# RFD-FHEM/PySignalduino

Measured on AMD Instinct MI355X. Metric: RF messages/sec demodulated (MU+MS+MC, full protocol bank), higher is better.
Workload: dtype u8+f64; 1 GPU; mixed MU/MS/MC stream, 1/3 each per rank: MU 256-pulse messages x 129-id MU bank, MS sync+bits x 66-id MS bank (clock x U(0.6,1.4)), MC frames x 12 clockrange ids ('fixed' chain); kind=mixed, corpus=bench, msgs_per_gpu=1000000, batches=3, input_bytes_resident=571611860, parallelism=dp1, grouped=True, streams=one kernel (k_step: MU, then MS, then MC tiles)

## Files before the change

### pysignalduino_amd/csrc/sdx_kernels.hip

```cpp
#include "sdx_device.h"
#include "sdx_lane.h"
#include "sdx_mc.h"

#include <atomic>
#include <cstdio>
#include <cstring>
#include <mutex>
#include <string>
#include <type_traits>

#ifdef SDX_WGTIME
__device__ unsigned long long g_wgt[2 * 65536];
#endif
#ifdef SDX_PROF
__device__ unsigned long long g_prof[32];
__device__ unsigned long long g_gprof[2][128];
#define PROF_T(v) unsigned long long v = __builtin_amdgcn_s_memtime()
#define PROF_ADD(slot, v)                                                                   \
  do {                                                                                      \
    if (__lane_id() == 0) L.prof[wave][slot] += (unsigned)(__builtin_amdgcn_s_memtime() - (v)); \
  } while (0)
#define PROF_CNT(slot, x)                                                                   \
  do {                                                                                      \
    if (__lane_id() == 0) L.prof[wave][slot] += (unsigned)(x);                              \
  } while (0)
#define PROF_ADDD(slot, v)                                                                  \
  do {                                                                                      \
    if (__lane_id() == __ffsll((unsigned long long)__builtin_amdgcn_read_exec()) - 1)       \
      L.prof[wave][slot] += (unsigned)(__builtin_amdgcn_s_memtime() - (v));                 \
  } while (0)
#define PROF_CNTL(slot) atomicAdd(&L.prof[wave][slot], 1u)
#else
#define PROF_T(v)
#define PROF_ADD(slot, v)
#define PROF_ADDD(slot, v)
#define PROF_CNT(slot, x)
#define PROF_CNTL(slot)
#endif

#ifndef SDX_NO_RAISE_CHECK
#define SDX_NO_RAISE_CHECK 1
#endif

namespace sdx {

constexpr int POOL_REC = 640;
constexpr int POOL_HEAP = 16384;
constexpr int POOL_REC_MS = 256;
constexpr int POOL_HEAP_MS = 8192;

struct StageRec {
  uint32_t off;
  uint16_t len, proto;
  uint32_t bitlen;
  uint8_t msg, wave;
  uint16_t rank;
};
constexpr uint32_t STAGE_NIB = 0x80000000u;
SDX_DEV uint32_t stage_bitlen(int bitlen, int hex_digits, int pre_len) {
  return (hex_digits >= 0 && hex_digits < 32768 && pre_len <= 255 && (uint32_t)bitlen < 65536u)
             ? (STAGE_NIB | ((uint32_t)hex_digits << 16) | (uint32_t)bitlen)
             : (uint32_t)bitlen;
}

struct MuItem {
  uint32_t st_lo, st_hi;
  uint16_t u0, u1, u2;
  uint16_t idx, p;
  uint8_t mi, fmask;
};
constexpr int QCAP = 128;
#ifndef SDX_LANE_WAVES
#define SDX_LANE_WAVES 8
#endif
constexpr int LANE_WAVES = SDX_LANE_WAVES;

struct MsItem {
  uint32_t k0_lo, k0_hi;
  uint16_t k1, k2, k3;
  uint16_t start;
  uint16_t p;
  uint8_t mi, fmask;
};
constexpr int MS_SURV_CAP = 1024;
constexpr int MS_DESC_LDS = 96;
struct MsDesc {
  int32_t lir_min, lir_max, pad, pre_off, post_off;
  uint16_t pre_len, post_len;
  uint8_t width, klen[4], recon, postdemo, res;
};
static_assert(sizeof(MsDesc) == 32, "MsDesc layout");

struct MuMatch {
  uint16_t q, k;
  uint16_t u0, u1, u2;
  uint16_t p;
  uint8_t mi;
  uint8_t flags;
  uint8_t j;
};
constexpr int MATCH_CAP = 768;

constexpr uint32_t SPILL_M = 2048, SPILL_R = 2048, SPILL_H = 49152;
constexpr uint32_t SPILL_OFF_R = SPILL_M * 16, SPILL_OFF_H = SPILL_OFF_R + SPILL_R * 16;
constexpr uint32_t SPILL_BYTES = SPILL_OFF_H + SPILL_H;
constexpr uint32_t SPILL_NONE = 0xFFFFFFFFu, SPILL_PENDING = 0xFFFFFFFEu, SPILL_FULL = 0xFFFFFFFDu;
constexpr uint32_t HEAP_SPILLED = 0x80000000u;
constexpr uint8_t REC_HOLE = 0xFF;
static_assert(sizeof(MuMatch) == 16, "MuMatch spill layout");

template <int NW, int TM, int LM>
struct TileLds {
  static constexpr int WS = NW;
  static constexpr int MSTRIDE = 10 * NW + 1;
  static constexpr int NBITS = 64 * NW + 64;
  struct Wave {
    uint64_t umask[3][NW];
    uint64_t uany[NW];
    uint64_t smask[NW];
    uint64_t stream[NW + 18];
    uint8_t bits[NBITS];
    uint8_t bits2[NBITS];
  };
  uint64_t bm[TM * MSTRIDE];
  uint64_t pairs[TM][2];
  int32_t nlen[TM];
  uint32_t raise_key[TM];
  uint32_t digit_ok[TM];
  uint32_t cnt[TM];
  uint32_t rec_base, heap_base, tile_bad, tot_rec;
  uint32_t mbase[TM];
  struct WaveScratch4 {
    Wave w[4];
  };
  struct NoScratch {};
  typename std::conditional<LM != 0, NoScratch, WaveScratch4>::type wa;
  static constexpr int PREC = LM == 1 ? 512 : (NW <= 4 ? POOL_REC_MS * (TM > 64 ? 2 : 1) : POOL_REC);
  static constexpr int PHEAP =
      LM == 1 ? 10240 : (NW <= 4 ? POOL_HEAP_MS * (TM > 64 ? 2 : 1) : POOL_HEAP);
  static constexpr int SCAP = TM > 64 ? MS_SURV_CAP + MS_SURV_CAP / 4 : MS_SURV_CAP;
  static constexpr int NHALF = (LM == 2 && TM > 64) ? 2 : 1;
  static_assert(TM <= 64 * NHALF, "one lane per message of a half");
  StageRec rec[PREC];
  alignas(16) uint8_t heap[PHEAP];
  unsigned long long pool_ctr;
  uint32_t spill_base, sp_rec, sp_heap;
  int ovf, next_p[NHALF];
  int mm_states, nmatch;
  MuMatch mlist[LM == 1 ? MATCH_CAP : 1];
  alignas(16) sdx_mu_desc desc[LM == 1 ? SDX_MUDESC_LDS : 1];
  union alignas(16) {
    MuItem q[LM == 1 ? LANE_WAVES : 1][LM == 1 ? QCAP : 1];
    uint8_t mmtab[LM == 1 ? SDX_MMTAB_LDS : 16];
  } u;
  MsItem slist[LM == 2 ? SCAP : 1];
  int nsurv;
  MsDesc msdesc[LM == 2 ? MS_DESC_LDS : 1];
#ifdef SDX_PROF
  unsigned int prof[LM != 0 ? LANE_WAVES : 4][28];
#endif
};

SDX_DEV void wave_sync() {
  __builtin_amdgcn_fence(__ATOMIC_SEQ_CST, "wavefront");
  __builtin_amdgcn_wave_barrier();
}

SDX_DEV int lanes_below(uint64_t mask) {
  const int l = lane_id();
  return popc64(l ? (mask & ((1ull << l) - 1)) : 0ull);
}

template <class T>
SDX_DEV int pool_alloc(T& L, int total, int* rec_slot) {
  int h = -1, r = -1;
  if (lane_id() == 0) {
    const unsigned long long o = atomicAdd(&L.pool_ctr, ((unsigned long long)total << 32) | 1ull);
    r = (int)(uint32_t)o;
    h = (int)(o >> 32);
    if (r >= T::PREC || h + total > T::PHEAP) {
      L.ovf = 1;
      h = -1;
    }
  }
  h = bcast_i(h, 0);
  *rec_slot = bcast_i(r, 0);
  return h;
}

template <class T>
SDX_DEV void pool_commit(T& L, int slot, int wave, int msg_local, int proto, int off, int total, int bitlen) {
  if (lane_id() == 0) {
    StageRec r;
    r.off = (uint32_t)off;
    r.len = (uint16_t)total;
    r.proto = (uint16_t)proto;
    r.bitlen = (uint32_t)bitlen;
    r.msg = (uint8_t)msg_local;
    r.wave = (uint8_t)wave;
    r.rank = (uint16_t)atomicAdd(&L.cnt[msg_local], 1u);
    L.rec[slot] = r;
  }
  wave_sync();
}

template <class T>
SDX_DEV uint32_t spill_region(T& L, const sdx_out& out) {
  uint32_t b = __hip_atomic_load(&L.spill_base, __ATOMIC_RELAXED, __HIP_MEMORY_SCOPE_WORKGROUP);
  if (b >= SPILL_PENDING) {
    const int leader = ffs64(ballot(true));
    if (lane_id() == leader) {
      uint32_t cur = atomicCAS(&L.spill_base, SPILL_NONE, SPILL_PENDING);
      if (cur == SPILL_NONE) {
        const uint32_t idx = atomicAdd(&out.cursor_dev[3], 1u);
        const uint64_t o = (uint64_t)idx * SPILL_BYTES;
        cur = (out.work_dev && o + SPILL_BYTES <= out.work_cap) ? (uint32_t)o : SPILL_FULL;
        __hip_atomic_store(&L.spill_base, cur, __ATOMIC_RELAXED, __HIP_MEMORY_SCOPE_WORKGROUP);
      }
      while (cur == SPILL_PENDING) cur = __hip_atomic_load(&L.spill_base, __ATOMIC_RELAXED, __HIP_MEMORY_SCOPE_WORKGROUP);
      b = cur;
    }
    b = (uint32_t)__shfl((int)b, leader);
  }
  if (b == SPILL_FULL || !out.work_dev || (uint64_t)b + SPILL_BYTES > out.work_cap) return SPILL_NONE;
  return b;
}

struct PoolSlot {
  StageRec* rec;
  uint8_t* heap;
  uint32_t off;
};
template <class T>
SDX_DEV bool pool_take(T& L, const sdx_out& out, int span, PoolSlot* ps) {
  const unsigned long long o = atomicAdd(&L.pool_ctr, ((unsigned long long)span << 32) | 1ull);
  const int slot = (int)(uint32_t)o, off = (int)(o >> 32);
  if (slot < T::PREC && off + span <= T::PHEAP) {
    ps->rec = &L.rec[slot];
    ps->heap = L.heap + off;
    ps->off = (uint32_t)off;
    return true;
  }
  if (slot < T::PREC) L.rec[slot].msg = REC_HOLE;
  const uint32_t base = spill_region(L, out);
  const uint32_t rs = atomicAdd(&L.sp_rec, 1u), hs = atomicAdd(&L.sp_heap, (uint32_t)span);
  if (base == SPILL_NONE || rs >= SPILL_R || hs + (uint32_t)span > SPILL_H) {
    L.ovf = 1;
    return false;
  }
  uint8_t* reg = out.work_dev + base;
  ps->rec = reinterpret_cast<StageRec*>(reg + SPILL_OFF_R) + rs;
  ps->heap = reg + SPILL_OFF_H + hs;
  ps->off = HEAP_SPILLED | hs;
  return true;
}

SDX_DEV void copy_str(uint8_t* dst, const uint8_t* src, int n) {
  for (int i = lane_id(); i < n; i += WAVE) dst[i] = src[i];
}

SDX_DEV int any_float(const uint8_t* bits, int nb) {
  bool f = false;
  for (int i = lane_id(); i < nb; i += WAVE) f |= bits[i] == 2;
  return ballot(f) != 0;
}

SDX_DEV int hex_digits(const uint8_t* bits, int nb, uint8_t* dst, int strip_zero) {
  const int nd = (nb + 3) >> 2;
  int skip = 0;
  if (strip_zero) {
    skip = nd;
    for (int d0 = 0; d0 < nd; d0 += WAVE) {
      const int d = d0 + lane_id();
      int v = 0;
      if (d < nd) {
        const int e = nb - 4 * (nd - 1 - d), a = (e - 4 > 0) ? e - 4 : 0;
        for (int i = a; i < e; ++i) v = (v << 1) | bits[i];
      }
      const uint64_t nz = ballot(d < nd && v != 0);
      if (nz) {
        skip = d0 + ffs64(nz);
        break;
      }
    }
  }
  for (int d = skip + lane_id(); d < nd; d += WAVE) {
    const int e = nb - 4 * (nd - 1 - d), a = (e - 4 > 0) ? e - 4 : 0;
    int v = 0;
    for (int i = a; i < e; ++i) v = (v << 1) | bits[i];
    dst[d - skip] = (uint8_t)(v < 10 ? '0' + v : 'A' + v - 10);
  }
  return nd - skip;
}

template <class T>
SDX_DEV void raise_msg(T& L, int msg_local, int proto, int kind) {
  if (lane_id() == 0) atomicMin(&L.raise_key[msg_local], ((uint32_t)proto << 8) | (uint32_t)kind);
  wave_sync();
}

template <int NW, int TM, int LM>
SDX_DEV void finish_mu(TileLds<NW, TM, LM>& L, int wave, const BankView& bv, const sdx_mu_proto* rec, int p, int s,
                       int nb) {
  auto& W = L.wa.w[wave];
  uint8_t* buf = W.bits;
  PROF_T(t_pd);
  if (cld(&rec->postdemo) != SDX_PD_NONE && !any_float(buf, nb)) {
    int rc = 0, no = 0;
    if (lane_id() == 0) rc = run_postdemo(cld(&rec->postdemo), buf, nb, W.bits2, &no);
    rc = bcast_i(rc, 0);
    no = bcast_i(no, 0);
    wave_sync();
    if (rc == 0) return;
    if (rc == 1) {
      buf = W.bits2;
      nb = no;
    }
  }
  PROF_ADD(7, t_pd);
  PROF_T(t_fmt);
  const int pad = cld(&rec->pad_bits);
  int nbp = nb;
  nbp = (nbp + pad - 1) / pad * pad;
  for (int i = nb + lane_id(); i < nbp; i += WAVE) buf[i] = 0;
  wave_sync();
  const bool isf = any_float(buf, nbp);
  int dlen;
  if (cld(&rec->dispatch_bin)) dlen = nbp;
  else if (isf) {
    if (cld(&rec->remove_zero)) {
      raise_msg(L, s, p, SDX_RAISE_ATTRIBUTE);
      return;
    }
    dlen = 4;
  } else {
    dlen = -2;
  }
  const int nd = (nbp + 3) >> 2;
  int skip = 0;
  if (dlen == -2) {
    if (cld(&rec->remove_zero)) {
      skip = nd;
      for (int d0 = 0; d0 < nd; d0 += WAVE) {
        const int d = d0 + lane_id();
        int v = 0;
        if (d < nd) {
          const int e = nbp - 4 * (nd - 1 - d), a = (e - 4 > 0) ? e - 4 : 0;
          for (int i = a; i < e; ++i) v = (v << 1) | buf[i];
        }
        const uint64_t nz = ballot(d < nd && v != 0);
        if (nz) {
          skip = d0 + ffs64(nz);
          break;
        }
      }
    }
    dlen = nd - skip;
  }
  auto dchar = [&](int d) -> uint8_t {
    if (cld(&rec->dispatch_bin)) return buf[d] == 2 ? 'F' : (uint8_t)('0' + buf[d]);
    if (isf) return (uint8_t)"None"[d];
    const int dd = d + skip, e = nbp - 4 * (nd - 1 - dd), a = (e - 4 > 0) ? e - 4 : 0;
    int v = 0;
    for (int i = a; i < e; ++i) v = (v << 1) | buf[i];
    return (uint8_t)(v < 10 ? '0' + v : 'A' + v - 10);
  };
  if (cld(&rec->mm_dfa) >= 0) {
    int ok = 0;
    if (lane_id() == 0) {
      const sdx_dfa D = bv.dfa[cld(&rec->mm_dfa)];
      const uint8_t* t256 = bv.t256 + D.t256_off;
      const uint8_t* fl = bv.dflags + D.flags_off;
      int st = cld(&rec->mm_pre_state);
      const int tot = dlen + cld(&rec->post_len);
      int i = 0;
      for (; i < tot; ++i) {
        const uint8_t f = fl[st];
        if (f & 5) break;
        const uint8_t c = i < dlen ? dchar(i) : bv.str[cld(&rec->post_off) + i - dlen];
        st = t256[st * 256 + c];
      }
      const uint8_t f = fl[st];
      ok = (f & 1) ? 1 : ((f & 4) ? 0 : ((i == tot && (f & 2)) ? 1 : 0));
    }
    PROF_ADD(9, t_fmt);
    if (!bcast_i(ok, 0)) return;
  }
  PROF_T(t_wr);
  const int total = cld(&rec->pre_len) + dlen + cld(&rec->post_len);
  int slot;
  const int off = pool_alloc(L, total, &slot);
  if (off < 0) return;
  uint8_t* dst = L.heap + off;
  copy_str(dst, bv.str + cld(&rec->pre_off), cld(&rec->pre_len));
  for (int d = lane_id(); d < dlen; d += WAVE) dst[cld(&rec->pre_len) + d] = dchar(d);
  copy_str(dst + cld(&rec->pre_len) + dlen, bv.str + cld(&rec->post_off), cld(&rec->post_len));
  pool_commit(L, slot, wave, s, p, off, total, (int)stage_bitlen(nbp, isf ? -1 : dlen, cld(&rec->pre_len)));
  PROF_ADD(8, t_wr);
  PROF_CNT(20, 1);
}

template <int NW, int TM, int LM>
SDX_DEV void decode_mu(TileLds<NW, TM, LM>& L, int wave, const BankView& bv, const sdx_mu_proto* rec, int p, int s,
                       int idx, uint64_t st_tgt, uint64_t ut0, uint64_t ut1, uint64_t ut2, int fmask) {
  using T = TileLds<NW, TM, LM>;
  auto& W = L.wa.w[wave];
  const int lane = lane_id();
  const uint64_t* bm = &L.bm[s * T::MSTRIDE];
  const int n = L.nlen[s], nw = (n + 63) >> 6;
  const int Lw = cld(&rec->width);
  const int lenS = cld(&rec->has_start) ? (int)cld(&rec->start.len) : 0;
  const uint64_t ut[3] = {ut0, ut1, ut2};
  const uint8_t SYM[3] = {1, 0, 2};
  PROF_T(t_setup);
  PROF_CNT(21, 1);
  uint64_t uni[3] = {0, 0, 0};
  uint8_t usym[3] = {0, 0, 0};
  int nu = 0;
  for (int k = 0; k < 3; ++k) {
    if (!((fmask >> k) & 1)) continue;
    int j = 0;
    for (; j < nu; ++j)
      if (uni[j] == ut[k]) break;
    if (j == nu) uni[nu++] = ut[k];
    usym[j] = SYM[k];
  }
  uint64_t ek[3] = {0, 0, 0};
  uint8_t esym[3] = {0, 0, 0};
  int ne = 0;
  if (cld(&rec->recon) && Lw > 1) {
    const uint64_t msk = (Lw - 1 >= 16) ? ~0ull : ((1ull << (4 * (Lw - 1))) - 1);
    for (int k = 0; k < 3; ++k) {
      if (!((fmask >> k) & 1)) continue;
      const uint64_t key = ut[k] & msk;
      int j = 0;
      for (; j < ne; ++j)
        if (ek[j] == key) break;
      if (j == ne) {
        ek[ne] = key;
        esym[ne] = SYM[k];
        ++ne;
      }
    }
  }
  if (lane < nw) {
    uint64_t any = 0;
    for (int j = 0; j < nu; ++j) {
      uint64_t m = ~0ull;
      for (int i = 0; i < Lw; ++i) {
        const int id = (int)((uni[j] >> (4 * i)) & 15), wo = lane + (i >> 6);
        m &= (wo < nw) ? bm_window(bm + id * T::WS, wo, i & 63, nw) : 0ull;
      }
      W.umask[j][lane] = m;
      any |= m;
    }
    W.uany[lane] = any;
    uint64_t sm = ~0ull;
    for (int i = 0; i < lenS; ++i) {
      const int id = (int)((st_tgt >> (4 * i)) & 15), wo = lane + (i >> 6);
      sm &= (wo < nw) ? bm_window(bm + id * T::WS, wo, i & 63, nw) : 0ull;
    }
    W.smask[lane] = sm;
  }
  wave_sync();
  const int nunits = (n + Lw - 1) / Lw;
  const int sw = (nunits + 63) >> 6;
  for (int r = 0; r < Lw; ++r) {
    for (int c = 0; c < sw; ++c) {
      const int x = r + (c * 64 + lane) * Lw;
      const bool b = x < n && ((W.uany[x >> 6] >> (x & 63)) & 1ull);
// ... 785 lines not shown
  __syncthreads();
  const uint32_t nh_l16 = ((uint32_t)nh_l + 15u) & ~15u;
  constexpr int MPL = (TM + 63) / 64;
  if (tid < 64) {
    const int lane = tid;
    uint32_t cm[MPL], c = 0;
#pragma unroll
    for (int k = 0; k < MPL; ++k) {
      const int m = lane * MPL + k;
      const bool live = !ovf && m < TM && m < nvalid && L.raise_key[m] == 0xFFFFFFFFu;
      cm[k] = live ? cntm[m] : 0u;
      c += cm[k];
    }
    uint32_t x = c;
#pragma unroll
    for (int o = 1; o < 64; o <<= 1) {
      const uint32_t y = __shfl_up(x, o);
      if (lane >= o) x += y;
    }
    uint32_t mb = x - c;
#pragma unroll
    for (int k = 0; k < MPL; ++k) {
      const int m = lane * MPL + k;
      if (m < TM && m < nvalid) L.mbase[m] = mb;
      mb += cm[k];
    }
    const uint32_t nrec = __shfl(x, 63);
    const uint32_t nheap = ovf ? 0u : nh_l16 + (((uint32_t)nh_s + 15u) & ~15u);
    uint32_t got = 0;
    if (!ovf && lane < 2) got = atomicAdd(&out.cursor_dev[lane], lane == 0 ? nrec : nheap);
    const uint32_t rb = __shfl(got, 0), hb = __shfl(got, 1);
    if (lane == 0) {
      int bad = ovf ? 1 : 0;
      if (!bad) {
        if (rb + nrec > out.rec_cap || hb + nheap > out.heap_cap) {
          bad = 2;
          atomicOr(&out.cursor_dev[2], 1u);
        }
      } else {
        atomicOr(&out.cursor_dev[2], 2u);
      }
      L.tile_bad = bad;
      L.rec_base = rb;
      L.heap_base = hb;
      L.tot_rec = nrec;
    }
  }
  __syncthreads();
  const int bad = L.tile_bad;
  if (!bad) {
    for (int r = tid; r < nr; r += blockDim.x) {
      const int m = rec_at(r).msg;
      if (m == REC_HOLE || L.raise_key[m] != 0xFFFFFFFFu) continue;
      const uint32_t b = atomicAdd(&fill[m], 1u);
      bidx[L.mbase[m] + b] = (uint16_t)r;
    }
    __syncthreads();
    const int nt = (int)L.tot_rec;
    for (int j = tid; j < nt; j += blockDim.x) {
      const StageRec sr = rec_at(bidx[j]);
      const uint32_t key = ((uint32_t)sr.proto << 16) | sr.rank;
      const uint32_t b0 = L.mbase[sr.msg], b1 = b0 + cntm[sr.msg];
      uint32_t rk = 0;
      for (uint32_t i = b0; i < b1; ++i) {
        const StageRec o = rec_at(bidx[i]);
        rk += (((uint32_t)o.proto << 16) | o.rank) < key ? 1u : 0u;
      }
      sdx_result o;
      o.payload_off = L.heap_base + ((sr.off & HEAP_SPILLED) ? nh_l16 + (sr.off & ~HEAP_SPILLED) : sr.off);
      o.payload_len = sr.len;
      o.proto = sr.proto;
      const bool staged_nib = (sr.bitlen & STAGE_NIB) != 0;
      o.bit_length = staged_nib ? (sr.bitlen & 0xFFFFu) : sr.bitlen;
      o.msg = (uint32_t)msg_of[sr.msg];
      out.rec_dev[L.rec_base + b0 + rk] = o;
      if (wx) {
        uint32_t xr;
        if (staged_nib) {
          const int pl = kind == SDX_KIND_MU ? bv.mu[sr.proto].pre_len : bv.ms[sr.proto].pre_len;
          xr = SDX_XREC_NIB | ((uint32_t)pl << 16) | ((sr.bitlen >> 16) & 0x7FFFu);
        } else if (sr.off & HEAP_SPILLED) {
          xr = wire_class(bv, kind, sr.proto, sreg + SPILL_OFF_H + (sr.off & ~HEAP_SPILLED), sr.len);
        } else {
          xr = wire_class(bv, kind, sr.proto, L.heap + sr.off, sr.len);
        }
        if (out.xrec_dev) out.xrec_dev[L.rec_base + b0 + rk] = xr;
        atomicAdd(reinterpret_cast<unsigned long long*>(&wsum[sr.msg]),
                  (unsigned long long)(((uint64_t)sr.len << 32) | wire_bytes_x(xr, sr.len)));
      }
    }
    uint8_t* hd = out.heap_dev + L.heap_base;
    if ((((uintptr_t)hd) & 15u) == 0) {
      const int n16 = (nh_l + 15) >> 4;
      const uint4* src = reinterpret_cast<const uint4*>(L.heap);
      uint4* dst = reinterpret_cast<uint4*>(hd);
      for (int i = tid; i < n16; i += blockDim.x) dst[i] = src[i];
      const int s16 = (nh_s + 15) >> 4;
      if (s16) {
        const uint4* ssrc = reinterpret_cast<const uint4*>(sreg + SPILL_OFF_H);
        uint4* sdst = reinterpret_cast<uint4*>(hd + nh_l16);
        for (int i = tid; i < s16; i += blockDim.x) sdst[i] = ssrc[i];
      }
    } else {
      for (int i = tid; i < nh_l; i += blockDim.x) hd[i] = L.heap[i];
      for (int i = tid; i < nh_s; i += blockDim.x) hd[nh_l16 + i] = sreg[SPILL_OFF_H + i];
    }
  }
  if (wx) __syncthreads();
  for (int m = tid; m < nvalid; m += blockDim.x) {
    sdx_desc d;
    d.rec_begin = L.rec_base + L.mbase[m];
    const uint32_t rk = L.raise_key[m];
    if (rk != 0xFFFFFFFFu) {
      d.status = SDX_ST_RAISED;
      d.raise_kind = (uint8_t)(rk & 0xFF);
      d.n_rec = 0;
    } else if (bad) {
      d.status = bad == 2 ? SDX_ST_OVF_OUT : SDX_ST_OVF_TILE;
      d.raise_kind = 0;
      d.n_rec = 0;
    } else {
      d.status = SDX_ST_OK;
      d.raise_kind = 0;
      d.n_rec = (uint16_t)cntm[m];
    }
    out.desc_dev[msg_of[m]] = d;
    if (wx) out.wire_dev[msg_of[m]] = d.status == SDX_ST_OK ? wsum[m] : 0ull;
  }
}

template <int KIND, int NW>
constexpr int pulses_threads() { return NW <= 4 ? 64 * LANE_WAVES : 256; }
template <int KIND, int NW>
constexpr int pulses_min_blocks() { return NW <= 4 ? 16 / LANE_WAVES : 1; }

template <int KIND, int NW, int TM>
using PulsesLds = TileLds<NW, TM, (KIND == SDX_KIND_MU && NW <= 4) ? 1 : ((KIND == SDX_KIND_MS && NW <= 4) ? 2 : 0)>;

template <int KIND, int NW, int TM, int MR, int SPLIT>
SDX_DEV void pulses_tile(const void* __restrict__ bank, const sdx_pulse_batch& b, const sdx_out& out, const int blk,
                         PulsesLds<KIND, NW, TM>& L, int* msg_of) {
  constexpr bool LANE_MU = KIND == SDX_KIND_MU && NW <= 4;
  constexpr bool LANE_MS = KIND == SDX_KIND_MS && NW <= 4;
  using T = PulsesLds<KIND, NW, TM>;
  const BankView bv = bank_view(bank);
  const int tid = threadIdx.x, wave = tid >> 6, lane = tid & 63;
  const int ntot = b.sel_dev ? b.n_sel : b.n;
  const int tile0 = blk * TM;
  const int nvalid = (ntot - tile0 < TM) ? ntot - tile0 : TM;
#ifdef SDX_WGTIME
  if (tid == 0 && blk < 65536) g_wgt[2 * blk] = __builtin_amdgcn_s_memrealtime();
#endif
  if constexpr (SPLIT != 0) {
    int len = 0;
    if (tid < nvalid) {
      const int msg = b.sel_dev ? b.sel_dev[tile0 + tid] : tile0 + tid;
      const int64_t o = b.offsets_dev[msg];
      len = b.len_dev ? b.len_dev[msg] : (int)(b.offsets_dev[msg + 1] - o);
    }
    const bool above = __syncthreads_or(len > 64 * NW) != 0;
    const bool below = SPLIT == 1 || __syncthreads_or(len > 64 * (SPLIT - 1)) != 0;
    if (above || !below) return;
  }
  if (tid < TM) {
    msg_of[tid] = (tid < nvalid) ? (b.sel_dev ? b.sel_dev[tile0 + tid] : tile0 + tid) : 0;
    L.raise_key[tid] = 0xFFFFFFFFu;
    L.cnt[tid] = 0;
  }
  if (tid == 0) {
#pragma unroll
    for (int h = 0; h < T::NHALF; ++h) L.next_p[h] = 0;
    L.nmatch = 0;
    L.pool_ctr = 0;
    L.spill_base = SPILL_NONE;
    L.sp_rec = 0;
    L.sp_heap = 0;
    L.ovf = 0;
    L.nsurv = 0;
  }
  if constexpr (LANE_MU) {
    const int ndesc = (int)bv.hdr->n_mu < SDX_MUDESC_LDS ? (int)bv.hdr->n_mu : SDX_MUDESC_LDS;
    const int n16 = (ndesc * (int)sizeof(sdx_mu_desc) + 15) >> 4;
    const uint4* src = reinterpret_cast<const uint4*>(bv.mudesc);
    uint4* dst = reinterpret_cast<uint4*>(L.desc);
    for (int i = tid; i < n16; i += blockDim.x) dst[i] = src[i];
    if (tid == 0) L.mm_states = (int)bv.hdr->mm_states;
  }
  if constexpr (LANE_MS) {
    const int nd = (int)bv.hdr->n_ms < MS_DESC_LDS ? (int)bv.hdr->n_ms : MS_DESC_LDS;
    for (int i = tid; i < nd; i += blockDim.x) L.msdesc[i] = ms_desc(bv.ms + i);
  }
#ifdef SDX_PROF
  if (lane < 28) L.prof[wave][lane] = 0;
#endif
  __syncthreads();
  PROF_T(t_kernel);
  PROF_T(t_stage);
  constexpr int NWAVE = pulses_threads<KIND, NW>() / 64;
  constexpr int MPW = NW <= 4 ? (TM + NWAVE - 1) / NWAVE : 1;
  static_assert(T::PHEAP >= TM * SDX_MAXPAT * 6 + TM * 16, "pattern staging fits the pool heap");
  uint32_t* st_x = reinterpret_cast<uint32_t*>(L.heap);
  uint8_t* st_f = L.heap + TM * SDX_MAXPAT * 4;
  uint8_t* st_id = st_f + TM * SDX_MAXPAT;
  double* st_clk = reinterpret_cast<double*>(st_id + TM * SDX_MAXPAT);
  uint8_t* st_np = reinterpret_cast<uint8_t*>(st_clk + TM);
  int64_t pf_off = 0;
  int pf_n = 0;
  constexpr int LPM = NW <= 4 ? 4 * NW : 16;
  constexpr int SMSG = 64 / LPM;
  constexpr int SPASS = (MPW + SMSG - 1) / SMSG;
  static_assert(NW > 4 || NW == 4 || NW == 2, "SWAR staging: 128- or 256-character rows");
  uint32_t sx[NW <= 4 ? SPASS : 1][5];
  if constexpr (NW <= 4) {
    const sdx_msg_rec* __restrict__ mrec = MR ? b.mrec_dev : nullptr;
    if (lane < MPW && wave + lane * NWAVE < nvalid) {
      const int msg = msg_of[wave + lane * NWAVE];
      if (mrec) {
        const int4 h = *reinterpret_cast<const int4*>(mrec + msg);
        pf_off = (int64_t)(((uint64_t)(uint32_t)h.y << 32) | (uint32_t)h.x);
        pf_n = h.z;
      } else {
        pf_off = b.offsets_dev[msg];
        pf_n = b.len_dev ? b.len_dev[msg] : (int)(b.offsets_dev[msg + 1] - pf_off);
      }
      if (pf_n > 64 * NW) pf_n = 64 * NW;
    }
    constexpr int NTH = pulses_threads<KIND, NW>();
    constexpr int NIT = (TM * SDX_MAXPAT + NTH - 1) / NTH;
    int r_np[NIT], r_cp[NIT];
    double r_v[NIT];
    uint8_t r_id[NIT];
    double2 r_all[NIT][KIND == SDX_KIND_MS ? SDX_MAXPAT / 2 : 1];
#pragma unroll
    for (int it = 0; it < NIT; ++it) {
      const int i = tid + it * NTH;
      const int m = i / SDX_MAXPAT, k = i - m * SDX_MAXPAT;
      const bool ok = i < TM * SDX_MAXPAT && m < nvalid;
      const int msg = ok ? msg_of[m] : 0;
      if (mrec) {
        const sdx_msg_rec* r = mrec + msg;
        r_np[it] = ok ? (int)r->npat : 0;
        r_v[it] = ok ? r->pat_val[k] : 0.0;
        r_id[it] = ok ? r->pat_id[k] : (uint8_t)'0';
      } else {
        r_np[it] = ok ? (int)b.npat_dev[msg] : 0;
        r_v[it] = ok ? b.pat_val_dev[msg * SDX_MAXPAT + k] : 0.0;
        r_id[it] = ok ? b.pat_id_dev[msg * SDX_MAXPAT + k] : (uint8_t)'0';
      }
      r_cp[it] = -1;
      if constexpr (KIND == SDX_KIND_MS) {
        r_cp[it] = ok ? (int)(mrec ? mrec[msg].cp_slot : b.cp_slot_dev[msg]) : -1;
        const double2* row = mrec ? reinterpret_cast<const double2*>(mrec[msg].pat_val)
                                  : reinterpret_cast<const double2*>(b.pat_val_dev + msg * SDX_MAXPAT);
#pragma unroll
        for (int h = 0; h < SDX_MAXPAT / 2; ++h) r_all[it][h] = ok ? row[h] : make_double2(0.0, 0.0);
      }
    }
#pragma unroll
    for (int it = 0; it < NIT; ++it) {
      const int i = tid + it * NTH;
      const int m = i / SDX_MAXPAT, k = i - m * SDX_MAXPAT;
      if (!(i < TM * SDX_MAXPAT && m < nvalid)) continue;
      const int np = r_np[it] > SDX_MAXPAT ? SDX_MAXPAT : r_np[it];
      if (k == 0) st_np[m] = (uint8_t)np;
      if (k >= np) continue;
      const double v = r_v[it];
      st_id[i] = (uint8_t)((r_id[it] - '0') & 15);
      if constexpr (KIND == SDX_KIND_MU) {
        const double av = fabs(v);
        const bool fast = av < 67108864.0 && av == floor(av);
        st_x[i] = fast ? (uint32_t)av * 10u : 0u;
        st_f[i] = (uint8_t)((signbit(v) ? 1 : 0) | (fast ? 0 : 2));
      } else {
        const int cp = r_cp[it];
        double pc = 0.0;
#pragma unroll
        for (int h = 0; h < SDX_MAXPAT / 2; ++h) {
          if (cp == 2 * h) pc = r_all[it][h].x;
          if (cp == 2 * h + 1) pc = r_all[it][h].y;
        }
        const double clk = (cp >= 0 && cp < np) ? fabs(pc) : 0.0;
        if (k == 0) st_clk[m] = clk;
        st_x[i] = (uint32_t)(clk != 0.0 ? py_round1_k(v / clk) : SDX_K_NONE);
      }
    }
    PROF_ADD(17, t_stage);
#pragma unroll
    for (int ps = 0; ps < SPASS; ++ps) {
      const int k = ps * SMSG + lane / LPM;
      const int lo = __shfl((int)(uint32_t)pf_off, k), hi = __shfl((int)(uint32_t)((uint64_t)pf_off >> 32), k);
      const int64_t off = (int64_t)(((uint64_t)(uint32_t)hi << 32) | (uint32_t)lo);
      const int n = __shfl(pf_n, k);
      const int64_t base = off + 16 * (lane % LPM);
      const int64_t a = base & ~(int64_t)3;
      const bool on = wave + k * NWAVE < nvalid;
      const uint32_t* src = reinterpret_cast<const uint32_t*>(b.data_dev + a);
#pragma unroll
      for (int i = 0; i < 5; ++i) sx[ps][i] = (on && a + 4 * i < off + n) ? src[i] : 0xFFFFFFFFu;
    }
  }
  PROF_T(t_bm);
  if constexpr (NW <= 4) {
  uint32_t ndmsg = 0;
#pragma unroll
  for (int ps = 0; ps < SPASS; ++ps) {
    const int k = ps * SMSG + lane / LPM, j = lane % LPM;
    const int mi = wave + k * NWAVE;
    const int n = __shfl(pf_n, k);
    const int lo = __shfl((int)(uint32_t)pf_off, k);
    const uint32_t r = (uint32_t)lo & 3u;
    uint32_t V = 0, P0 = 0, P1 = 0, P2 = 0, P3 = 0, FE = 0;
#pragma unroll
    for (int i = 0; i < 4; ++i) {
      uint32_t c = __builtin_amdgcn_alignbyte(sx[ps][i + 1], sx[ps][i], r);
      const int rem = n - (16 * j + 4 * i);
      c = rem >= 4 ? c : (rem <= 0 ? 0xFFFFFFFFu : (c | (0xFFFFFFFFu << (8 * rem))));
      const uint32_t t = c ^ 0x30303030u;
      const uint32_t lo4 = t & 0x0F0F0F0Fu;
      const uint32_t bad = (t & 0xF0F0F0F0u) | ((lo4 + 0x06060606u) & 0x10101010u);
      const uint32_t nz = ((bad & 0x7F7F7F7Fu) + 0x7F7F7F7Fu) | bad;
      const uint32_t dg = (~nz >> 7) & 0x01010101u;
      V |= ((dg * 0x01020408u) >> 24) << (4 * i);
      P0 |= (((lo4 & 0x01010101u) * 0x01020408u) >> 24) << (4 * i);
      P1 |= (((lo4 & 0x02020202u) * 0x00810204u) >> 24) << (4 * i);
      P2 |= (((lo4 & 0x04040404u) * 0x00408102u) >> 24) << (4 * i);
      P3 |= (((lo4 & 0x08080808u) * 0x00204081u) >> 24) << (4 * i);
      if (__builtin_expect(bad != 0 && rem > 0, 0)) {
        const uint32_t fe = c ^ 0xFEFEFEFEu;
        const uint32_t fz = ~(((fe & 0x7F7F7F7Fu) + 0x7F7F7F7Fu) | fe) & 0x80808080u;
        FE |= ((((fz >> 7) & 0x01010101u) * 0x01020408u) >> 24) << (4 * i);
      }
    }
    const uint32_t posm = n - 16 * j >= 16 ? 0xFFFFu : (n - 16 * j <= 0 ? 0u : (1u << (n - 16 * j)) - 1u);
    const bool nondigit = (posm & ~V & ~FE) != 0;
    const uint64_t ndb = ballot(nondigit);
#pragma unroll
    for (int g = 0; g < SMSG; ++g)
      if ((ndb >> (LPM * g)) & ((1ull << LPM) - 1)) ndmsg |= 1u << (ps * SMSG + g);
    if (mi < nvalid) {
      const uint32_t N0 = ~P0, N1 = ~P1, N2 = ~P2, N3 = ~P3;
      uint16_t* row = reinterpret_cast<uint16_t*>(&L.bm[mi * T::MSTRIDE + (j >> 2)]) + (j & 3);
#pragma unroll
      for (int id = 0; id < 10; ++id) {
        const uint32_t m = V & ((id & 1) ? P0 : N0) & ((id & 2) ? P1 : N1) & ((id & 4) ? P2 : N2) &
                           ((id & 8) ? P3 : N3);
        row[id * T::WS * 4] = (uint16_t)m;
      }
    }
  }
  wave_sync();
  PROF_ADD(18, t_bm);
  PROF_T(t_pairs);
#pragma unroll
  for (int k = 0; k < MPW; ++k) {
    const int mi = wave + k * NWAVE;
    if (mi >= nvalid) break;
    const int n = __shfl(pf_n, k);
    const int nwu = (n + 63) >> 6;
    const uint64_t nd = (ndmsg >> k) & 1u;
    if constexpr (NW <= 4) {
      wave_sync();
      uint64_t pr[2];
#pragma unroll
      for (int h = 0; h < 2; ++h) {
        const int q = lane + 64 * h;
        uint64_t acc = 0;
        if (q < 100) {
          const uint64_t* A = &L.bm[mi * T::MSTRIDE + (q / 10) * T::WS];
          const uint64_t* B = &L.bm[mi * T::MSTRIDE + (q % 10) * T::WS];
#pragma unroll
          for (int w = 0; w < NW; ++w)
            if (KIND != SDX_KIND_MS || w < nwu) acc |= A[w] & ((B[w] >> 1) | (w + 1 < NW ? B[w + 1] << 63 : 0ull));
        }
        pr[h] = ballot(acc != 0);
      }
      if (lane == 0) {
        L.pairs[mi][0] = pr[0];
        L.pairs[mi][1] = pr[1];
      }
    }
    if (lane == 0) {
      L.nlen[mi] = n;
      L.digit_ok[mi] = (nd == 0 && n > 0) ? 1u : 0u;
    }
  }
  PROF_ADD(19, t_pairs);
  }
  if constexpr (NW > 4) {
    for (int mi = wave; mi < nvalid; mi += NWAVE) {
      const int msg = msg_of[mi];
      const int64_t off = b.offsets_dev[msg];
      int n = b.len_dev ? b.len_dev[msg] : (int)(b.offsets_dev[msg + 1] - off);
      if (n > 64 * NW) n = 64 * NW;
      bool nondigit = false;
      for (int w = 0; w < NW; ++w) {
        const int pos = w * 64 + lane;
        const uint8_t c = pos < n ? b.data_dev[off + pos] : (uint8_t)0xFF;
        nondigit |= pos < n && !((c >= '0' && c <= '9') || c == 0xFE);
        uint64_t mine = 0;
#pragma unroll
        for (int id = 0; id < 10; ++id) {
          const uint64_t bb = ballot(c == (uint8_t)('0' + id));
          if (lane == id) mine = bb;
        }
        if (lane < 10) L.bm[mi * T::MSTRIDE + lane * T::WS + w] = mine;
      }
      const uint64_t nd = ballot(nondigit);
      if (lane == 0) {
        L.nlen[mi] = n;
        L.digit_ok[mi] = (nd == 0 && n > 0) ? 1u : 0u;
      }
    }
  }
  __syncthreads();
  PROF_ADD(0, t_stage);
  const int half = T::NHALF > 1 ? wave / (NWAVE / T::NHALF) : 0;
  const int mi = lane + 64 * half;
  const bool mvalid = mi < nvalid;
  int npat = 0, n = 0;
  uint64_t ids = 0;
  double val[SDX_MAXPAT];
  int kq[SDX_MAXPAT];
#pragma unroll
  for (int k = 0; k < SDX_MAXPAT; ++k) {
    val[k] = 0.0;
    kq[k] = SDX_K_NONE;
  }
  bool lane_ok = false;
  uint32_t xk[SDX_MAXPAT];
  uint32_t negm = 0, slowm = 0;
#pragma unroll
  for (int k = 0; k < SDX_MAXPAT; ++k) xk[k] = 0;
  if (mvalid) {
    const int msg = msg_of[mi];
    if constexpr (NW <= 4) {
      npat = st_np[mi];
#pragma unroll
      for (int k = 0; k < SDX_MAXPAT; ++k) {
        if (k < npat) {
          const int i = mi * SDX_MAXPAT + k;
          ids |= (uint64_t)st_id[i] << (4 * k);
          if constexpr (LANE_MU) {
            xk[k] = st_x[i];
            const uint32_t f = st_f[i];
            negm |= (f & 1u) << k;
            slowm |= ((f >> 1) & 1u) << k;
          } else {
            kq[k] = (int)st_x[i];
          }
        }
      }
    } else {
      npat = b.npat_dev[msg];
      if (npat > SDX_MAXPAT) npat = SDX_MAXPAT;
#pragma unroll
      for (int k = 0; k < SDX_MAXPAT; ++k) {
        if (k < npat) {
          ids |= (uint64_t)((b.pat_id_dev[msg * SDX_MAXPAT + k] - '0') & 15) << (4 * k);
          val[k] = b.pat_val_dev[msg * SDX_MAXPAT + k];
        }
      }
    }
    n = L.nlen[mi];
    lane_ok = n > 0;
  }
  PairRef PR{0, 0};
  if constexpr (NW <= 4) {
    if (mvalid) {
      PR.P0 = L.pairs[mi][0];
      PR.P1 = L.pairs[mi][1];
    }
  }
  const uint64_t* bmine = &L.bm[(mvalid ? mi : 0) * T::MSTRIDE];
  const int nw = (n + 63) >> 6;
  double clock = 0.0;
  if (KIND == SDX_KIND_MS && mvalid) {
    const int msg = msg_of[mi];
    const bool use_rec = MR && NW <= 4;
    const int cp = use_rec ? b.mrec_dev[msg].cp_slot : b.cp_slot_dev[msg];
    const bool ok_ms = use_rec ? b.mrec_dev[msg].ms_ok : b.ms_ok_dev[msg];
    lane_ok = lane_ok && L.digit_ok[mi] && ok_ms && cp >= 0 && cp < npat;
    if constexpr (NW <= 4) {
      clock = st_clk[mi];
      lane_ok = lane_ok && clock != 0.0;
      if (!lane_ok) {
#pragma unroll
        for (int k = 0; k < SDX_MAXPAT; ++k) kq[k] = SDX_K_NONE;
      }
    } else {
#pragma unroll
      for (int k = 0; k < SDX_MAXPAT; ++k)
        if (k == cp) clock = fabs(val[k]);
      lane_ok = lane_ok && clock != 0.0;
      if (lane_ok) {
#pragma unroll
        for (int k = 0; k < SDX_MAXPAT; ++k)
          if (k < npat) kq[k] = py_round1_k(val[k] / clock);
      }
    }
  }
  auto PEXV = [&](const SpecV& sv, const sdx_patspec* sp, int minpos, bool need_pos) -> PexRes {
    if constexpr (NW <= 4) return pexists_lane<NW>(sv, kq, ids, npat, bmine, minpos, bv.rank, PR, need_pos);
    else return pattern_exists(sp, kq, ids, npat, bmine, T::WS, nw, minpos);
  };
  const int nproto = KIND == SDX_KIND_MU ? (int)bv.hdr->n_mu : (int)bv.hdr->n_ms;
  const uint16_t* order = bv.order + (KIND == SDX_KIND_MU ? 0 : (int)bv.hdr->n_mu);
  double last_clock = __builtin_nan("");
  MuItem* Q = nullptr;
  int q_head = 0, q_tail = 0;
  if constexpr (LANE_MU) Q = L.u.q[wave];
  auto drain = [&](int head, int cnt) {
    wave_sync();
    if constexpr (KIND == SDX_KIND_MU && NW <= 4) {
      if (lane < cnt) {
        const MuItem it = Q[(head + lane) & (QCAP - 1)];
        const int qm = it.mi, qp = it.p;
        const uint32_t rk = L.raise_key[qm];
        if (rk == 0xFFFFFFFFu || (rk >> 8) > (uint32_t)qp) {
          sdx_mu_desc d;
          if (qp < SDX_MUDESC_LDS) d = L.desc[qp];
          else d = bv.mudesc[qp];
          PROF_CNTL(21);
          decode_mu_lane<NW>(L, out, wave, bv, bv.mu + qp, d, qp, qm, &L.bm[qm * T::MSTRIDE], L.nlen[qm], it.idx,
                             ((uint64_t)it.st_hi << 32) | it.st_lo, it.u0, it.u1, it.u2, it.fmask);
        }
      }
    }
    wave_sync();
  };
  const int ngrab = KIND == SDX_KIND_MU ? (int)bv.hdr->n_mu_groups : nproto;
  const uint16_t* gstart = bv.order + bv.hdr->n_mu + bv.hdr->n_ms;
  int cur = 0, cend = 0;
#ifdef SDX_PROF
  int g_cur = -1;
  unsigned long long g_t0 = 0;
#endif
  while (true) {
    if (cur == cend) {
      int g = 0;
      if (lane == 0) g = atomicAdd(&L.next_p[half], 1);
      g = __builtin_amdgcn_readfirstlane(g);
#ifdef SDX_PROF
      if (g_cur >= 0 && g_cur < 128 && lane == 0) {
        atomicAdd(&g_gprof[0][g_cur], __builtin_amdgcn_s_memtime() - g_t0);
        atomicAdd(&g_gprof[1][g_cur], 1ull);
      }
      g_cur = g;
      g_t0 = __builtin_amdgcn_s_memtime();
#endif
      if (g >= ngrab || (T::NHALF > 1 && 64 * half >= nvalid)) break;
      if (KIND == SDX_KIND_MU) {
        cur = cld(&gstart[g]);
        cend = cld(&gstart[g + 1]);
      } else {
        cur = g;
        cend = g + 1;
      }
    }
    const int p = cld(&order[cur]);
    ++cur;
    if constexpr (KIND == SDX_KIND_MU) {
      const sdx_mu_proto* rec = uniform_ptr(bv.mu + p);
      const sdx_mu_filt* fr = uniform_ptr(bv.mufilt + p);
      const uint32_t ff = cld(&fr->flags);
      if ((ff & 2u) || !(ff & 4u)) continue;
      const bool full = (ff & 8u) != 0;
      bool alive = lane_ok && (SDX_NO_RAISE_CHECK || (L.raise_key[mi] >> 8) > (uint32_t)p || L.raise_key[mi] == 0xFFFFFFFFu);
      int idx = 0;
      uint64_t st_tgt = 0, ut0 = 0, ut1 = 0, ut2 = 0;
      int fmask = 0;
      PROF_T(t_norm);
      const double pclk = cld(&fr->clock);
      if (pclk != last_clock) {
        last_clock = pclk;
        if constexpr (LANE_MU) {
          const uint32_t csh = cld(&fr->clk_sh);
          const uint32_t cc = cld(&fr->clk_c), cm = cld(&fr->clk_m), sh = csh & 0xFFu;
          const bool ivalid = (csh & 0x100u) != 0, cneg = (csh & 0x200u) != 0;
#pragma unroll
          for (int k = 0; k < SDX_MAXPAT; ++k) {
            if (k < npat) {
              const bool slow = !ivalid || ((slowm >> k) & 1u);
              const bool negk = ((negm >> k) & 1u) != 0;
              int kk = 0;
              if (!slow) {
                const uint32_t x = xk[k];
                const uint32_t q = (uint32_t)(((uint64_t)x * cm) >> sh);
                const int d2 = 2 * (int)(x - q * cc) - (int)cc;
                kk = (int)q + (d2 > 0 ? 1 : 0);
                if (d2 == 0) kk = py_round1_k((double)(2 * q + 1) / 20.0);
                if (negk != cneg) kk = -kk;
              }
              if (slow) kk = py_round1_k(b.pat_val_dev[msg_of[mi] * SDX_MAXPAT + k] / pclk);
              kq[k] = kk;
            }
          }
        } else {
#pragma unroll
          for (int k = 0; k < SDX_MAXPAT; ++k)
            if (k < npat) kq[k] = py_round1_k(val[k] / pclk);
        }
      }
      PROF_ADD(1, t_norm);
      auto SV = [&](int key, const sdx_patspec* sp) -> SpecV {
        if constexpr (NW <= 4) {
          if (!full) return spec_compact(&fr->spec[key], key == 0 ? cld(&fr->start_upk) : (uint64_t)cld(&fr->spec[key].upk));
          return spec_full(sp);
        } else {
          return SpecV{};
        }
      };
      PROF_T(t_st);
      if (alive) {
        if (ff & 1u) {
          const PexRes r = PEXV(SV(0, &rec->start), &rec->start, 0, true);
          alive = r.found;
          idx = r.pos;
          st_tgt = r.tgt;
        }
      }
      PROF_ADD(2, t_st);
      PROF_T(t_ozf);
      auto klen = [&](int key) -> int { return (int)((cld(&fr->spec[key].rk2_len_nu) >> 16) & 0xFF); };
      if (alive && klen(1)) {
        const PexRes r = PEXV(SV(1, &rec->one), &rec->one, idx, false);
        if (r.found) { ut0 = r.tgt; fmask |= 1; } else alive = false;
      }
      if (alive && klen(2)) {
        const PexRes r = PEXV(SV(2, &rec->zero), &rec->zero, idx, false);
        if (r.found) { ut1 = r.tgt; fmask |= 2; } else alive = false;
      }
      if (alive && klen(3)) {
        const PexRes r = PEXV(SV(3, &rec->flt), &rec->flt, idx, false);
        if (r.found) { ut2 = r.tgt; fmask |= 4; }
      }
      alive = alive && fmask != 0;
      PROF_ADD(3, t_ozf);
      PROF_T(t_dec);
      if constexpr (NW <= 4) {
        const uint64_t pass = ballot(alive);
        if (pass) {
          if (alive) {
            MuItem it;
            it.st_lo = (uint32_t)st_tgt;
            it.st_hi = (uint32_t)(st_tgt >> 32);
            it.u0 = (uint16_t)ut0;
            it.u1 = (uint16_t)ut1;
            it.u2 = (uint16_t)ut2;
            it.idx = (uint16_t)idx;
            it.p = (uint16_t)p;
            it.mi = (uint8_t)mi;
            it.fmask = (uint8_t)fmask;
            Q[(q_tail + lanes_below(pass)) & (QCAP - 1)] = it;
          }
          q_tail += popc64(pass);
          if (q_tail - q_head >= WAVE) {
            drain(q_head, WAVE);
            q_head += WAVE;
          }
        }
      } else {
        uint64_t surv = ballot(alive);
        while (surv) {
          const int sl = ffs64(surv);
          surv &= surv - 1;
          decode_mu(L, wave, bv, rec, p, sl, bcast_i(idx, sl), bcast_u64(st_tgt, sl), bcast_u64(ut0, sl),
                    bcast_u64(ut1, sl), bcast_u64(ut2, sl), bcast_i(fmask, sl));
        }
      }
      PROF_ADD(12, t_dec);
    } else {
      const sdx_ms_proto* rec = uniform_ptr(bv.ms + p);
      const sdx_ms_filt* fr = uniform_ptr(bv.msfilt + p);
      const uint32_t ff = cld(&fr->flags);
      if (ff & 2u) continue;
      const bool full = (ff & 8u) != 0;
      bool alive = lane_ok && ((LANE_MS && SDX_NO_RAISE_CHECK) || (L.raise_key[mi] >> 8) > (uint32_t)p ||
                               L.raise_key[mi] == 0xFFFFFFFFu);
      const double pclk = cld(&fr->pclock);
      if (alive && pclk > 0.0)
        alive = !(fabs(pclk - clock) > clock * 0.3);
      int start = 0;
      uint64_t kt0 = 0, kt1 = 0, kt2 = 0, kt3 = 0;
      int fmask = 0;
      auto SV = [&](int key) -> SpecV {
        if constexpr (NW <= 4) {
          if (!full) return spec_compact(&fr->spec[key], key == 0 ? cld(&fr->sync_upk) : (uint64_t)cld(&fr->spec[key].upk));
          return spec_full(&rec->key[key]);
// ... 1218 lines not shown
```

Measured before the change: 677.4 million msgs/s.

## Compute digit-pair presence masks in registers with DPP reductions instead of LDS bitmaps

For short messages, the set of adjacent digit pairs is now built directly in registers. Each lane takes its nibbles and the following byte, forms an index pair*10+next, sets bits in a 100-bit mask, and ORs the masks across the lane group with DPP row shuffles. This replaces the second pass, which re-read the per-digit bitmaps from LDS and ran 100 shifted AND comparisons with ballots per message. The old path is kept behind SDX_PAIRS_LDS. In exchange, each lane uses more registers and needs correct handling of pairs that cross lane-group boundaries, via the fifth loaded word.

Measured after the change: 700.5 million msgs/s (median of 6 runs). 1.03x the previous value.

```diff
diff --git a/pysignalduino_amd/csrc/sdx_kernels.hip b/pysignalduino_amd/csrc/sdx_kernels.hip
--- a/pysignalduino_amd/csrc/sdx_kernels.hip
+++ b/pysignalduino_amd/csrc/sdx_kernels.hip
@@ -166,6 +166,16 @@
   __builtin_amdgcn_wave_barrier();
 }
 
+template <int G>
+SDX_DEV uint32_t group_or(uint32_t v) {
+  static_assert(G == 8 || G == 16, "a half row or a row of 16 lanes");
+  v |= (uint32_t)__builtin_amdgcn_update_dpp(0, (int)v, 0xB1, 0xF, 0xF, true);
+  v |= (uint32_t)__builtin_amdgcn_update_dpp(0, (int)v, 0x4E, 0xF, 0xF, true);
+  v |= (uint32_t)__builtin_amdgcn_update_dpp(0, (int)v, 0x141, 0xF, 0xF, true);
+  if constexpr (G == 16) v |= (uint32_t)__builtin_amdgcn_update_dpp(0, (int)v, 0x140, 0xF, 0xF, true);
+  return v;
+}
+
 SDX_DEV int lanes_below(uint64_t mask) {
   const int l = lane_id();
   return popc64(l ? (mask & ((1ull << l) - 1)) : 0ull);
@@ -1557,6 +1567,9 @@
   PROF_T(t_bm);
   if constexpr (NW <= 4) {
   uint32_t ndmsg = 0;
+#ifdef SDX_PROF
+  unsigned long long pair_cy = 0;
+#endif
 #pragma unroll
   for (int ps = 0; ps < SPASS; ++ps) {
     const int k = ps * SMSG + lane / LPM, j = lane % LPM;
@@ -1565,6 +1578,9 @@
     const int lo = __shfl((int)(uint32_t)pf_off, k);
     const uint32_t r = (uint32_t)lo & 3u;
     uint32_t V = 0, P0 = 0, P1 = 0, P2 = 0, P3 = 0, FE = 0;
+#ifndef SDX_PAIRS_LDS
+    uint32_t l4[5], dgt[5];
+#endif
 #pragma unroll
     for (int i = 0; i < 4; ++i) {
       uint32_t c = __builtin_amdgcn_alignbyte(sx[ps][i + 1], sx[ps][i], r);
@@ -1575,6 +1591,10 @@
       const uint32_t bad = (t & 0xF0F0F0F0u) | ((lo4 + 0x06060606u) & 0x10101010u);
       const uint32_t nz = ((bad & 0x7F7F7F7Fu) + 0x7F7F7F7Fu) | bad;
       const uint32_t dg = (~nz >> 7) & 0x01010101u;
+#ifndef SDX_PAIRS_LDS
+      l4[i] = lo4;
+      dgt[i] = dg;
+#endif
       V |= ((dg * 0x01020408u) >> 24) << (4 * i);
       P0 |= (((lo4 & 0x01010101u) * 0x01020408u) >> 24) << (4 * i);
       P1 |= (((lo4 & 0x02020202u) * 0x00810204u) >> 24) << (4 * i);
@@ -1602,10 +1622,56 @@
         row[id * T::WS * 4] = (uint16_t)m;
       }
     }
+#ifndef SDX_PAIRS_LDS
+    {
+#ifdef SDX_PROF
+      const unsigned long long t_p0 = __builtin_amdgcn_s_memtime();
+#endif
+      const uint32_t ct = ((sx[ps][4] >> (8 * r)) & 0xFFu) ^ 0x30u;
+      l4[4] = ct & 15u;
+      dgt[4] = (ct < 10u && 16 * j + 16 < n) ? 1u : 0u;
+      uint64_t plo = 0, phi = 0;
+#pragma unroll
+      for (int i = 0; i < 4; ++i) {
+        const uint32_t nx = __builtin_amdgcn_alignbyte(l4[i + 1], l4[i], 1);
+        const uint32_t vd = dgt[i] & __builtin_amdgcn_alignbyte(dgt[i + 1], dgt[i], 1);
+        const uint32_t q4 = (l4[i] * 10u + nx) | ((vd ^ 0x01010101u) * 0xFFu);
+#pragma unroll
+        for (int e = 0; e < 4; ++e) {
+          const uint32_t q = (q4 >> (8 * e)) & 0xFFu;
+          const uint64_t bit = 1ull << (q & 63u);
+          const uint64_t up = 0ull - (uint64_t)((q >> 6) & 1u);
+          plo |= bit & ~up;
+          phi |= bit & up;
+        }
+      }
+      uint32_t pw[4] = {(uint32_t)plo, (uint32_t)(plo >> 32), (uint32_t)phi, (uint32_t)(phi >> 32) & 0xFu};
+#pragma unroll
+      for (int w = 0; w < 4; ++w) pw[w] = group_or<LPM>(pw[w]);
+      if (j == 0 && mi < nvalid) {
+        L.pairs[mi][0] = ((uint64_t)pw[1] << 32) | pw[0];
+        L.pairs[mi][1] = ((uint64_t)pw[3] << 32) | pw[2];
+        L.nlen[mi] = n;
+        L.digit_ok[mi] = (((ndb >> (lane & ~(LPM - 1))) & ((1ull << LPM) - 1)) == 0 && n > 0) ? 1u : 0u;
+      }
+#ifdef SDX_PROF
+      pair_cy += __builtin_amdgcn_s_memtime() - t_p0;
+#endif
+    }
+#endif
   }
   wave_sync();
+#ifdef SDX_PAIRS_LDS
   PROF_ADD(18, t_bm);
   PROF_T(t_pairs);
+#else
+  (void)ndmsg;
+#ifdef SDX_PROF
+  PROF_ADD(18, t_bm + pair_cy);
+  const unsigned long long t_pairs = __builtin_amdgcn_s_memtime() - pair_cy;
+#endif
+#endif
+#ifdef SDX_PAIRS_LDS
 #pragma unroll
   for (int k = 0; k < MPW; ++k) {
     const int mi = wave + k * NWAVE;
@@ -1639,6 +1705,7 @@
       L.digit_ok[mi] = (nd == 0 && n > 0) ? 1u : 0u;
     }
   }
+#endif
   PROF_ADD(19, t_pairs);
   }
   if constexpr (NW > 4) {
```
